# srihari-humbarwadi/retinanet-tensorflow2.x

Hardware: AMD Instinct MI355X
Metric: images/sec train, ResNet50-640 RetinaNet data-parallel step (encode + fwd + loss + bwd + clip + all-reduce + SGD/EMA); inference images/s under `infer` (higher is better)
Workload: dtype bf16; 1 GPU; ResNet50-640x640 bf16 training, 32 images/GPU (BASELINE configs[2] shard: global batch 32), resnet_initial frozen, single GPU; global_batch=32, parallelism=dp1, rccl_ranks=1, comm=torch, syncbn_messages=0

## Files before the change

retinanet-tensorflow2.x_amd/csrc/rn_conv_big.hip:

```cpp
#include "rn_conv_big_epi.h"

namespace {

constexpr int BM = 256, BN = 256, BK = 32, NW = 8, STAGES = 4;
constexpr int A_BYTES = BM * BK * 2, STAGE_BYTES = (BM + BN) * BK * 2;
constexpr int RING_BYTES = STAGES * STAGE_BYTES, PATCH_BYTES = 4096;
constexpr int LDS_BYTES = RING_BYTES + NW * PATCH_BYTES;

template <bool OUT_F32, bool HAS_RES, bool BN_BWD = false>
__global__ void __launch_bounds__(512) conv_big_kernel(const ConvArgs args) {
  extern __shared__ __attribute__((aligned(16))) char smem[];
  const int total = args.total_tiles;
  const int G = gridDim.x;
  const int tid = threadIdx.x;
  const int lane = tid & 63;
  const int wave = __builtin_amdgcn_readfirstlane(tid >> 6);
  const int wave_m = wave >> 2, wave_n = wave & 3;
  const int R = args.R, S = args.S, RS = R * S;

  int i_v = blockIdx.x;
  int i_tap = 0, i_c0 = 0;
  int i_r = 0, i_s = 0;
  int g_iss = 0;
  int i_W = 0, i_PS = 0, i_Cin = 0, i_cw = 0;
  __amdgpu_buffer_rsrc_t rs_x, rs_w;
  unsigned a_off[2], a_mask[2], b_off[2];
  const int d_row = lane >> 2, d_pos = lane & 3;

#define BIG_SETUP_ISSUE()                                                                             \
  do {                                                                                                \
    const int tile__ = (args.pad_ & 2) ? i_v : tile_of(i_v, total);      \
    int si__ = 0;                                                                                     \
    _Pragma("unroll 1") for (int i = 1; i < args.nseg; ++i)                                           \
      if (tile__ >= args.seg[i].tile_begin) si__ = i;                                                 \
    const ConvSegDev& sg__ = args.seg[si__];                                                          \
    const int lt__ = tile__ - sg__.tile_begin;                                                        \
    const int mt__ = rn_fdiv(lt__, sg__.n_tiles, rn_rcp((float)sg__.n_tiles));   \
    const int rows_t__ = sg__.rows ? sg__.rows : BM;      \
    const int m0__ = mt__ * rows_t__, n0__ = (lt__ - mt__ * sg__.n_tiles) * BN;                       \
    const int mend__ = m0__ + rows_t__ < sg__.M ? m0__ + rows_t__ : sg__.M;                           \
    i_W = sg__.W; i_PS = sg__.pix_stride; i_Cin = sg__.CinP; i_cw = sg__.cwrap;                       \
    const int H__ = sg__.H, Ktot__ = RS * i_Cin;                                                      \
    const int rows__ = sg__.Cout <= 64 ? 64 : ((sg__.Cout + 127) / 128) * 128;  \
    rs_x = __builtin_amdgcn_make_buffer_rsrc((void*)sg__.x, 0,                                        \
                                             (int)((long long)sg__.N * H__ * i_W * i_PS * 2), 0x00020000); \
    rs_w = __builtin_amdgcn_make_buffer_rsrc((void*)sg__.w, 0, (int)((long long)rows__ * Ktot__ * 2), \
                                             0x00020000);                                             \
    const float rWo__ = rn_rcp((float)sg__.Wo), rHo__ = rn_rcp((float)sg__.Ho);                 \
    _Pragma("unroll") for (int j = 0; j < 2; ++j) {                                                   \
      const int row = (j * NW + wave) * 16 + d_row;                                                   \
      const int chunk = d_pos ^ lds_swz<BK>(row);                                                     \
      const int m = m0__ + row;                                                                       \
      const int mm = m < mend__ ? m : 0;                                                              \
      int ox, oy, n;                                                                                  \
      if (args.pad_ & 1) {    \
        const int t2 = rn_fdiv(mm, sg__.Wo, rWo__);                                                   \
        ox = mm - t2 * sg__.Wo;                                                                       \
        n = rn_fdiv(t2, sg__.Ho, rHo__);                                                              \
        oy = t2 - n * sg__.Ho;                                                                        \
      } else {                                                                                        \
        ox = mm % sg__.Wo;                                                                            \
        const int t2 = mm / sg__.Wo;                                                                  \
        oy = t2 % sg__.Ho;                                                                            \
        n = t2 / sg__.Ho;                                                                             \
      }                                                                                               \
      const int iy0 = oy * args.sh - args.pt, ix0 = ox * args.sw - args.pl;                           \
      a_off[j] = (unsigned)(((((long long)n * H__ + iy0) * i_W + ix0) * i_PS + chunk * 8) * 2);       \
      unsigned mask = 0;                                                                              \
      if (m < mend__) {                                                                               \
        for (int r = 0; r < R; ++r)                                                                   \
          for (int s = 0; s < S; ++s) {                                                               \
            const bool ok = (unsigned)(iy0 + r) < (unsigned)H__ && (unsigned)(ix0 + s) < (unsigned)i_W; \
            mask |= (ok ? 1u : 0u) << (r * S + s);                                                    \
          }                                                                                           \
      }                                                                                               \
      a_mask[j] = mask;                                                                               \
      const int nrow = n0__ + row;                                                                    \
      b_off[j] = nrow < rows__ ? (unsigned)(((long long)nrow * Ktot__ + chunk * 8) * 2) : RN_OOB;     \
    }                                                                                                 \
  } while (0)

#define BIG_ISSUE_STEP()                                                                              \
  do {                                                                                                \
    const int cw__ = i_c0 < i_cw ? i_c0 : (i_c0 < 2 * i_cw ? i_c0 - i_cw : i_c0 - 2 * i_cw);          \
    const unsigned tap_off__ = (unsigned)((((long long)i_r * i_W + i_s) * i_PS + cw__) * 2);          \
    const unsigned koff__ = (unsigned)(((long long)i_tap * i_Cin + i_c0) * 2);                        \
    char* st__ = smem + (g_iss & 3) * STAGE_BYTES;                                                    \
    _Pragma("unroll") for (int j = 0; j < 2; ++j) {                                                   \
      const unsigned v__ = ((a_mask[j] >> i_tap) & 1u) ? a_off[j] + tap_off__ : RN_OOB;               \
      dma16(rs_x, st__ + (j * NW + wave) * 1024, v__);                                                \
    }                                                                                                 \
    _Pragma("unroll") for (int j = 0; j < 2; ++j)                                                     \
      dma16(rs_w, st__ + A_BYTES + (j * NW + wave) * 1024, b_off[j] == RN_OOB ? RN_OOB : b_off[j] + koff__); \
    ++g_iss;                                                                                          \
    i_c0 += BK;                                                                                       \
    if (i_c0 >= i_Cin) {                                                                              \
      i_c0 = 0;                                                                                       \
      ++i_tap;                                                                                        \
      if (++i_s == S) {                                                                               \
        i_s = 0;                                                                                      \
        ++i_r;                                                                                        \
      }                                                                                               \
      if (__builtin_expect(i_tap == RS, 0)) {                                                         \
        i_tap = i_r = i_s = 0;                                                                        \
        i_v += G;                                                                                     \
        if (i_v < total) BIG_SETUP_ISSUE();                                                           \
      }                                                                                               \
    }                                                                                                 \
  } while (0)

  int off_p0, off_w0;
  {
    const int fr = lane & 31, fh = lane >> 5;
    const int sw = (fr >> 2) & 3;
    off_p0 = (wave_m * 128 + fr) * 64 + ((0 + fh) ^ sw) * 16;
    off_w0 = A_BYTES + (wave_n * 64 + fr) * 64 + ((0 + fh) ^ sw) * 16;
  }

  f32x16_t acc[4][2];
#pragma unroll
  for (int i = 0; i < 4; ++i)
#pragma unroll
    for (int j = 0; j < 2; ++j)
#pragma unroll
      for (int r = 0; r < 16; ++r) acc[i][j][r] = 0.0f;

  bf16x8_t px0[4], wt0[2], px1[4], wt1[2];
#define BIG_READ(stage_)                                                                              \
  do {                                                                                                \
    const char* b__ = smem + (stage_) * STAGE_BYTES;                                                  \
    _Pragma("unroll") for (int j = 0; j < 2; ++j) wt0[j] = *(const bf16x8_t*)(b__ + off_w0 + j * 2048); \
    _Pragma("unroll") for (int i = 0; i < 4; ++i) px0[i] = *(const bf16x8_t*)(b__ + off_p0 + i * 2048); \
    _Pragma("unroll") for (int j = 0; j < 2; ++j) wt1[j] = *(const bf16x8_t*)(b__ + (off_w0 ^ 32) + j * 2048); \
    _Pragma("unroll") for (int i = 0; i < 4; ++i) px1[i] = *(const bf16x8_t*)(b__ + (off_p0 ^ 32) + i * 2048); \
  } while (0)
#define BIG_LOADSEG(stage_)                                                                           \
  do {                                                                                                \
    BIG_READ(stage_);                                                                                 \
    if (i_v < total) {                                                                                \
      BIG_ISSUE_STEP();                                                                               \
      asm volatile("s_waitcnt vmcnt(8)" ::: "memory");                                                \
    } else {                                                                                          \
      asm volatile("s_waitcnt vmcnt(0)" ::: "memory");                                                \
    }                                                                                                 \
    asm volatile("s_waitcnt lgkmcnt(0)" ::: "memory");                                                \
  } while (0)
#define BIG_COMPUTESEG()                                                                              \
  do {                                                                                                \
    __builtin_amdgcn_sched_barrier(0);                                                                \
    _Pragma("unroll") for (int i = 0; i < 4; ++i)                                                     \
      _Pragma("unroll") for (int j = 0; j < 2; ++j)                                                   \
        acc[i][j] = RN_MFMA_32x32x16(wt0[j], px0[i], acc[i][j], 0, 0, 0);      \
    _Pragma("unroll") for (int i = 0; i < 4; ++i)                                                     \
      _Pragma("unroll") for (int j = 0; j < 2; ++j)                                                   \
        acc[i][j] = RN_MFMA_32x32x16(wt1[j], px1[i], acc[i][j], 0, 0, 0);      \
    __builtin_amdgcn_sched_barrier(0);                                                                \
  } while (0)
#define BIG_BARRIER()                       \
  do {                                      \
    __builtin_amdgcn_s_barrier();           \
    asm volatile("" ::: "memory");          \
  } while (0)

  int c_v = blockIdx.x;
  int c_k = 0;
  int c_ksteps, c_m0, c_n0, c_si, c_mend, c_chunk0;
#define BIG_SETUP_COMPUTE()                                                                           \
  do {                                                                                                \
    const int tile__ = (args.pad_ & 2) ? c_v : tile_of(c_v, total);                                   \
    c_si = 0;                                                                                         \
    _Pragma("unroll 1") for (int i = 1; i < args.nseg; ++i)                                           \
      if (tile__ >= args.seg[i].tile_begin) c_si = i;                                                 \
    const ConvSegDev& sg__ = args.seg[c_si];                                                          \
    const int lt__ = tile__ - sg__.tile_begin;                                                        \
    const int mt__ = rn_fdiv(lt__, sg__.n_tiles, rn_rcp((float)sg__.n_tiles));   \
    const int rows_t__ = sg__.rows ? sg__.rows : BM;                                                  \
    c_m0 = mt__ * rows_t__;                                                                           \
    c_mend = c_m0 + rows_t__ < sg__.M ? c_m0 + rows_t__ : sg__.M;                                     \
    c_chunk0 = mt__ * 2;                                                                              \
    c_n0 = (lt__ - mt__ * sg__.n_tiles) * BN;                                                         \
    c_ksteps = RS * (sg__.CinP / BK);                                                                 \
    c_k = 0;                                                                                          \
  } while (0)

  auto epilogue = [&]() __attribute__((always_inline)) {
    big_epilogue<OUT_F32, HAS_RES, BN_BWD>(acc, args, c_si, c_m0, c_n0, wave, smem + RING_BYTES + wave * PATCH_BYTES,
                                           BigEpiSrc(), c_mend, c_chunk0);
  };

  BIG_SETUP_ISSUE();
  BIG_SETUP_COMPUTE();
  big_acc_init<OUT_F32, HAS_RES>(acc, args, c_si, c_n0, wave);
#pragma unroll 1
  for (int t = 0; t < 3 && i_v < total; ++t) BIG_ISSUE_STEP();
  if (g_iss >= 3) asm volatile("s_waitcnt vmcnt(4)" ::: "memory");
  else asm volatile("s_waitcnt vmcnt(0)" ::: "memory");
  BIG_BARRIER();
  BIG_LOADSEG(0);
  if (wave_m == 1) BIG_BARRIER();

#define BIG_TILE_END()                                       \
  if (__builtin_expect(c_k == c_ksteps, 0)) {               \
    epilogue();                                             \
    if (c_v + G >= total) break;                            \
    c_v += G;                                               \
    BIG_SETUP_COMPUTE();                                    \
    big_acc_init<OUT_F32, HAS_RES>(acc, args, c_si, c_n0, wave); \
  }
  int g = 0;
#pragma unroll 1
  while (true) {
    BIG_COMPUTESEG();
    ++c_k;
    if (wave_m == 0) BIG_BARRIER();
    BIG_TILE_END();
    if (wave_m == 1) BIG_BARRIER();
    ++g;
    BIG_LOADSEG(g & 3);
    BIG_BARRIER();
  }
#undef BIG_TILE_END
#undef BIG_SETUP_COMPUTE
#undef BIG_BARRIER
#undef BIG_COMPUTESEG
#undef BIG_LOADSEG
#undef BIG_READ
#undef BIG_ISSUE_STEP
#undef BIG_SETUP_ISSUE
}

}

int rn_launch_conv_big(const ConvArgs& a, bool out_f32, const rn_launch_opts& opts, hipStream_t st) {
  static unsigned long long attr_set = 0;
  if (RN_ATTRS_NEEDED(attr_set)) {
    RN_CHECK_HIP(hipFuncSetAttribute((const void*)conv_big_kernel<false, false>,
                                     hipFuncAttributeMaxDynamicSharedMemorySize, LDS_BYTES));
    RN_CHECK_HIP(hipFuncSetAttribute((const void*)conv_big_kernel<false, true>,
                                     hipFuncAttributeMaxDynamicSharedMemorySize, LDS_BYTES));
    RN_CHECK_HIP(hipFuncSetAttribute((const void*)conv_big_kernel<true, false>,
                                     hipFuncAttributeMaxDynamicSharedMemorySize, LDS_BYTES));
    RN_CHECK_HIP(hipFuncSetAttribute((const void*)conv_big_kernel<true, true>,
                                     hipFuncAttributeMaxDynamicSharedMemorySize, LDS_BYTES));
    RN_CHECK_HIP(hipFuncSetAttribute((const void*)conv_big_kernel<false, false, true>,
                                     hipFuncAttributeMaxDynamicSharedMemorySize, LDS_BYTES));
    RN_ATTRS_DONE(attr_set);
  }
  const int grid = rn_persistent_grid(a.total_tiles, rn_num_cus(), opts);
  bool has_res = false;
  for (int i = 0; i < a.nseg; ++i) has_res = has_res || a.seg[i].residual != nullptr;
  const dim3 g3(grid), b3(512);
  if (a.seg[0].bn_y) {
    hipLaunchKernelGGL((conv_big_kernel<false, false, true>), g3, b3, LDS_BYTES, st, a);
  } else if (out_f32) {
    if (has_res) hipLaunchKernelGGL((conv_big_kernel<true, true>), g3, b3, LDS_BYTES, st, a);
    else hipLaunchKernelGGL((conv_big_kernel<true, false>), g3, b3, LDS_BYTES, st, a);
  } else {
    if (has_res) hipLaunchKernelGGL((conv_big_kernel<false, true>), g3, b3, LDS_BYTES, st, a);
    else hipLaunchKernelGGL((conv_big_kernel<false, false>), g3, b3, LDS_BYTES, st, a);
  }
  RN_CHECK_LAUNCH();
  return RN_OK;
}
```

retinanet-tensorflow2.x_amd/csrc/rn_conv_dispatch.hip:

```cpp
#include <algorithm>
#include <map>
#include <mutex>
#include <tuple>

#include "rn_conv_dev.h"

extern "C" int rn_conv_cout_pad(int Cout) { return Cout <= 64 ? 64 : (int)rn_align_up((size_t)Cout, 128); }
extern "C" int rn_conv_cin_pad(int Cin) { return Cin <= 32 ? 32 : (int)rn_align_up((size_t)Cin, 64); }
extern "C" int rn_conv_pair_rows(int Cout) { return Cout > 0 ? 128 * ((Cout + 63) / 64) : 0; }

struct ConvPlanSeg {
  int cols, cols_pad;
  int terms, cin_pad;
  long long M;
  int n_tiles, tile_begin;
  int bn_row_blocks;
};

struct ConvPlan {
  int kid;
  int BM, BN;
  int BK;
  int bal_rows;
  bool deal;
  bool fast_div;
  int order[RN_CONV_MAX_SEGMENTS];
  long long total_tiles;
  int min_depth;
  int split_parts;
  long long ws_bytes;
  ConvPlanSeg seg[RN_CONV_MAX_SEGMENTS];
};

static long long seg_tiles(const ConvPlanSeg& s, int rows, int width) { return rn_cdiv(s.M, rows) * rn_cdiv(s.cols_pad, width); }
static long long conv_tiles(const ConvPlan& pl, int nseg, int rows, int width) {
  long long t = 0;
  for (int i = 0; i < nseg; ++i) t += seg_tiles(pl.seg[i], rows, width);
  return t;
}

static bool conv_halo_fits(const rn_conv_problem* p, int BM) {
  if (p->opts.conv_no_halo) return false;
  if (p->R != 3 || p->S != 3 || p->stride_h != 1 || p->stride_w != 1 || p->pad_top != 1 || p->pad_left != 1)
    return false;
  static std::mutex mu;
  static std::map<std::tuple<int, int, int, int>, int> patch_px;
  for (int i = 0; i < p->num_segments; ++i) {
    const rn_conv_segment& s = p->seg[i];
    if (s.Ho != s.H || s.Wo != s.W || s.Cin % 32 != 0) return false;
    if ((long long)s.N * s.H * s.W >= (1ll << 22)) return false;
    std::lock_guard<std::mutex> lock(mu);
    const auto key = std::make_tuple(s.N, s.H, s.W, BM);
    auto it = patch_px.find(key);
    if (it == patch_px.end()) it = patch_px.emplace(key, rn_conv_halo_patch_pixels(s.N, s.H, s.W, rn_conv_halo_pitch(s.W), BM)).first;
    if (it->second > rn_conv_halo_capacity(BM)) return false;
  }
  return true;
}

static int splitk_parts(int total, int min_chunks, int G0, long long* bytes) {
  const int L = total % G0;
  if (bytes) *bytes = 0;
  if (L == 0 || L > 511 || min_chunks < 8) return 1;
  int S = G0 / L;
  if (S > min_chunks / 4) S = min_chunks / 4;
  if (S > 4) S = 4;
  if (S < 2) return 1;
  if (bytes) *bytes = RN_SPLITK_HEADER_BYTES + (long long)L * S * RN_SPLITK_SLOT_BYTES;
  return S;
}

static void rn_splitk_plan(ConvArgs& a, int min_chunks, void* ws, long long ws_bytes, const rn_launch_opts& opts) {
  const int total = a.total_tiles;
  a.split_f = total; a.split_s = 1; a.vtotal = total; a.pad2_ = 0; a.ws = nullptr;
  const int G0 = rn_persistent_grid(0x7fffffff, rn_num_cus(), opts);
  const int L = total % G0;
  int S = ws ? splitk_parts(total, min_chunks, G0, nullptr) : 1;
  while (S >= 2 && RN_SPLITK_HEADER_BYTES + (long long)L * S * RN_SPLITK_SLOT_BYTES > ws_bytes) --S;
  if (S < 2) return;
  a.split_f = total - L; a.split_s = S; a.vtotal = L * S; a.ws = (float*)ws;
}

extern "C" size_t rn_conv_splitk_workspace_max_bytes(void) { return RN_SPLITK_HEADER_BYTES + 256ull * RN_SPLITK_SLOT_BYTES; }

static int conv_big_balanced_rows(const rn_conv_problem* p, const ConvPlanSeg& s) {
  if (p->num_segments != 1 || p->R != 1 || p->S != 1 || p->stride_h != 1 || p->stride_w != 1) return 0;
  if (p->opts.conv_tile || p->opts.conv_big_min_tiles || p->opts.max_workgroups || p->splitk_ws) return 0;
  if (s.terms * s.cin_pad > 512) return 0;
  const int n_tiles = (int)rn_cdiv(s.cols_pad, 256);
  const int G = rn_persistent_grid(0x7fffffff, rn_num_cus(), p->opts);
  const long long T = seg_tiles(s, 256, 256);
  if (T <= 0 || G <= 0) return 0;
  const long long rounds = rn_cdiv(T, G);
  const long long m_tiles = rounds * G / n_tiles;
  if (m_tiles < 1) return 0;
  long long rows = rn_cdiv(s.M, m_tiles);
  rows = (rows + 3) / 4 * 4;
  if (rows < 64 || rows > 236) return 0;
  return (int)rows;
}

#define RN_SPLIT128_MIN_STEPS 4
static int conv128_split_parts(const rn_launch_opts& opts, long long tiles, int ksteps, int BN, long long ws_bytes) {
  if (opts.conv_tile == 1 || tiles < 1 || tiles > 4096) return 1;
  const int target = opts.splitk_target_blocks > 0 ? opts.splitk_target_blocks : rn_num_cus() * 3 / 4;
  int S = target / (int)tiles;
  if (S > ksteps / RN_SPLIT128_MIN_STEPS) S = ksteps / RN_SPLIT128_MIN_STEPS;
  if (S > 8) S = 8;
  const long long slot = 128ll * BN * 4;
  while (S >= 2 && RN_SPLITK_HEADER_BYTES + tiles * S * slot > ws_bytes) --S;
  return S >= 2 ? S : 1;
}

static bool conv_plan(const rn_conv_problem* p, bool assume_ws, ConvPlan& pl) {
  if (!p || p->num_segments < 1 || p->num_segments > RN_CONV_MAX_SEGMENTS) return false;
  const int nseg = p->num_segments;
  const rn_launch_opts& o = p->opts;

  bool all_wide = true, all_128 = true, all_128s_or_64 = true, one_col = true;
  bool epi_ok = true;
  long long dmin = 1ll << 60, dmax = 0;
  pl.min_depth = 0x7fffffff;
  pl.fast_div = true;
  for (int i = 0; i < nseg; ++i) {
    const rn_conv_segment& s = p->seg[i];
    ConvPlanSeg& d = pl.seg[i];
    d.cols = s.w_pair ? rn_conv_pair_rows(s.Cout) : s.Cout;
    d.cols_pad = rn_conv_cout_pad(d.cols);
    d.terms = s.w_terms > 1 ? s.w_terms : 1;
    d.cin_pad = rn_conv_cin_pad(s.Cin);
    d.M = (long long)s.N * s.Ho * s.Wo;
    all_wide = all_wide && d.cols_pad >= 256;
    all_128 = all_128 && d.cols_pad == 128;
    all_128s_or_64 = all_128s_or_64 && (d.cols_pad % 128 == 0 || d.cols_pad == 64);
    one_col = one_col && d.cols_pad <= 256;
    epi_ok = epi_ok && s.Cout % (p->out_dtype == RN_DT_F32 && s.w_pair ? 4 : 8) == 0 && !(s.bias && s.residual);
    const int depth = d.terms * d.cin_pad;
    pl.min_depth = depth < pl.min_depth ? depth : pl.min_depth;
    const long long depth_all = (long long)p->R * p->S * d.cin_pad * d.terms;
    dmin = depth_all < dmin ? depth_all : dmin;
    dmax = depth_all > dmax ? depth_all : dmax;
    pl.fast_div = pl.fast_div && d.M < (1 << 22);
  }
  const int cin0 = pl.seg[0].cin_pad;
  pl.BK = (cin0 % 64 != 0 || (long long)p->R * p->S * cin0 <= 256) ? 32 : 64;

  const bool use_big = o.conv_tile != 1 && o.conv_tile != 3 && all_wide && epi_ok &&
                       (o.conv_tile == 2 || conv_tiles(pl, nseg, 256, 256) >= (o.conv_big_min_tiles > 0 ? o.conv_big_min_tiles : 192));
  if (use_big) {
    if (!conv_halo_fits(p, 256)) pl.kid = 1;
    else pl.kid = (o.conv_tile == 0 && o.conv_big_min_tiles == 0 && conv_halo_fits(p, 512)) ? 3 : 2;
  } else {
    const bool halo512 = o.conv_tile != 1 && !o.conv_no_halo && (o.conv_tile == 3 ? all_128s_or_64 : all_128) && epi_ok &&
                         (o.conv_tile >= 2 || conv_tiles(pl, nseg, 512, 128) >= (o.conv_big_min_tiles > 0 ? o.conv_big_min_tiles : 128)) &&
                         conv_halo_fits(p, 512);
    pl.kid = halo512 ? 3 : 0;
  }

  pl.bal_rows = 0;
  if (pl.kid == 0) {
    pl.BM = 128;
    pl.BN = pl.seg[0].cols_pad <= 64 ? 64 : 128;
    if (pl.BN == 128 && o.conv_tile != 1 && 2 * conv_tiles(pl, nseg, 128, 128) <= rn_num_cus()) pl.BN = 64;
  } else if (pl.kid == 3) {
    pl.BM = 512; pl.BN = 128;
  } else {
    pl.BM = 256; pl.BN = 256;
    if (pl.kid == 1) pl.bal_rows = conv_big_balanced_rows(p, pl.seg[0]);
  }

  for (int i = 0; i < nseg; ++i) pl.order[i] = i;
  pl.deal = pl.kid == 1 && nseg > 1 && one_col && dmax >= 2 * dmin;
  if (pl.deal)
    std::stable_sort(pl.order, pl.order + nseg, [&](int x, int y) {
      return pl.seg[x].cin_pad * pl.seg[x].terms > pl.seg[y].cin_pad * pl.seg[y].terms;
    });
  const int rows = pl.bal_rows ? pl.bal_rows : pl.BM;
  pl.total_tiles = 0;
  for (int ii = 0; ii < nseg; ++ii) {
    ConvPlanSeg& d = pl.seg[pl.order[ii]];
    d.n_tiles = (int)rn_cdiv(d.cols_pad, pl.BN);
    d.tile_begin = (int)pl.total_tiles;
    d.bn_row_blocks = (int)(pl.bal_rows ? 2 * rn_cdiv(d.M, rows) : (rows / 128) * rn_cdiv(d.M, rows));
    pl.total_tiles += seg_tiles(d, rows, pl.BN);
  }

  pl.split_parts = 1;
  pl.ws_bytes = 0;
  if (pl.kid == 0) {
    if (p->splitk_ws || assume_ws) {
      const long long avail = p->splitk_ws ? p->splitk_ws_bytes : (long long)rn_conv_splitk_workspace_max_bytes();
      pl.split_parts = conv128_split_parts(o, pl.total_tiles, p->R * p->S * (pl.min_depth / pl.BK), pl.BN, avail);
    }
    if (pl.split_parts >= 2) pl.ws_bytes = RN_SPLITK_HEADER_BYTES + pl.total_tiles * pl.split_parts * 128 * pl.BN * 4;
  } else if (pl.kid == 2) {
    splitk_parts((int)pl.total_tiles, pl.min_depth / 32, rn_persistent_grid(0x7fffffff, rn_num_cus(), o), &pl.ws_bytes);
  }
  return true;
}

extern "C" size_t rn_conv_splitk_workspace_bytes(const rn_conv_problem* p) {
  ConvPlan pl;
  return conv_plan(p, true, pl) ? (size_t)pl.ws_bytes : 0;
}

extern "C" int rn_conv_kernel_id(const rn_conv_problem* p) {
  ConvPlan pl;
  return conv_plan(p, false, pl) ? pl.kid : -1;
}

extern "C" int rn_conv_bn_row_blocks(const rn_conv_problem* p, int segment) {
  ConvPlan pl;
  if (!conv_plan(p, false, pl) || segment < 0 || segment >= p->num_segments) return 0;
  return pl.seg[segment].bn_row_blocks;
}

extern "C" int rn_conv_tile_rows(const rn_conv_problem* p) {
  ConvPlan pl;
  return conv_plan(p, false, pl) ? pl.BM : 0;
}

static int conv_validate(const rn_conv_problem* p, const ConvPlan& pl) {
  RN_CHECK_ARG(p->R >= 1 && p->S >= 1 && p->R * p->S <= 32, "rn_conv2d_nhwc_fwd: R*S=%d > 32", p->R * p->S);
  RN_CHECK_ARG(p->stride_h >= 1 && p->stride_w >= 1, "rn_conv2d_nhwc_fwd: bad stride");
  RN_CHECK_ARG(p->out_dtype == RN_DT_BF16 || p->out_dtype == RN_DT_F32, "rn_conv2d_nhwc_fwd: bad out_dtype");
  if (const int orc = rn_validate_launch_opts(p->opts, "rn_conv2d_nhwc_fwd")) return orc;
  for (int ii = 0; ii < p->num_segments; ++ii) {
    const int i = pl.order[ii];
    const rn_conv_segment& s = p->seg[i];
    RN_CHECK_ARG(s.x && s.w && s.y, "rn_conv2d_nhwc_fwd: segment %d has a null tensor", i);
    RN_CHECK_ARG(s.N > 0 && s.H > 0 && s.W > 0 && s.Ho > 0 && s.Wo > 0 && s.Cout > 0 && s.Cin > 0,
                 "rn_conv2d_nhwc_fwd: segment %d bad shape", i);
    RN_CHECK_ARG(s.Cin % 8 == 0 && pl.seg[i].cin_pad % pl.BK == 0,
                 "rn_conv2d_nhwc_fwd: segment %d Cin=%d must be a multiple of 8 (K step %d)", i, s.Cin, pl.BK);
    RN_CHECK_ARG(s.pix_stride % 4 == 0 && s.pix_stride > 0,
                 "rn_conv2d_nhwc_fwd: segment %d pix_stride=%d must be a positive multiple of 4", i, s.pix_stride);
    RN_CHECK_ARG(s.Cout % 4 == 0, "rn_conv2d_nhwc_fwd: segment %d Cout=%d not a multiple of 4", i, s.Cout);
    RN_CHECK_ARG((pl.seg[i].cols_pad <= 64) == (pl.seg[0].cols_pad <= 64), "rn_conv2d_nhwc_fwd: segments mix Cout tile widths");
    RN_CHECK_ARG(!s.w_pair || (pl.kid != 0 && p->out_dtype == RN_DT_F32 && s.w_terms <= 1 && !s.scale && !s.shift &&
                               !s.residual && !s.bn_partial),
                 "rn_conv2d_nhwc_fwd: segment %d: w_pair needs an f32 launch without scale / shift / residual that the 256- / "
                 "512-row kernels take (rn_conv_kernel_id() != 0)", i);
    RN_CHECK_ARG(((uintptr_t)s.x | (uintptr_t)s.w | (uintptr_t)s.y | (uintptr_t)s.residual) % 16 == 0,
                 "rn_conv2d_nhwc_fwd: segment %d tensors must be 16-byte aligned", i);
    RN_CHECK_ARG(pl.seg[i].M < (1ll << 31) && (long long)s.N * s.H * s.W * s.pix_stride * 2 < (1ll << 31),
                 "rn_conv2d_nhwc_fwd: segment %d input exceeds the 2 GiB buffer-addressing limit", i);
    if (s.bn_bwd_y) {
      RN_CHECK_ARG(s.bn_partial && s.bn_bwd_fwd && p->out_dtype == RN_DT_BF16 && !s.scale && !s.shift && !s.bias &&
                       !s.residual && p->act == RN_ACT_NONE && s.Cout % 8 == 0 && (uintptr_t)s.bn_bwd_y % 16 == 0,
                   "rn_conv2d_nhwc_fwd: segment %d: bn_bwd_y needs bn_partial + bn_bwd_fwd on a plain bf16 launch", i);
    }
    RN_CHECK_ARG((s.bn_bwd_y != nullptr) == (p->seg[0].bn_bwd_y != nullptr),
                 "rn_conv2d_nhwc_fwd: bn_bwd_y must be set on all segments or none");
    RN_CHECK_ARG(pl.seg[i].terms <= 3, "rn_conv2d_nhwc_fwd: segment %d w_terms=%d (1..3)", i, s.w_terms);
  }
  RN_CHECK_ARG(p->splitk_ws == nullptr || ((uintptr_t)p->splitk_ws % 16 == 0 && p->splitk_ws_bytes >= 0),
               "rn_conv2d_nhwc_fwd: splitk_ws must be 16-byte aligned");
  return RN_OK;
}

extern "C" int rn_conv2d_nhwc_fwd(const rn_conv_problem* p, void* stream) {
  RN_CHECK_ARG(p != nullptr, "rn_conv2d_nhwc_fwd: null problem");
  RN_CHECK_ARG(p->num_segments >= 1 && p->num_segments <= RN_CONV_MAX_SEGMENTS,
               "rn_conv2d_nhwc_fwd: num_segments=%d", p->num_segments);
  ConvPlan pl;
  conv_plan(p, false, pl);
  if (const int rc = conv_validate(p, pl)) return rc;

  ConvArgs a;
  a.R = p->R; a.S = p->S; a.sh = p->stride_h; a.sw = p->stride_w; a.pt = p->pad_top; a.pl = p->pad_left;
  a.act = p->act; a.nseg = p->num_segments;
  a.total_tiles = (int)pl.total_tiles;
  a.pad_ = pl.kid <= 1 ? (pl.fast_div ? 1 : 0) | (pl.deal ? 2 : 0) : 0;
  a.split_f = a.vtotal = a.total_tiles; a.split_s = 1; a.pad2_ = 0; a.ws = nullptr;
  for (int ii = 0; ii < p->num_segments; ++ii) {
    const rn_conv_segment& s = p->seg[pl.order[ii]];
    const ConvPlanSeg& ps = pl.seg[pl.order[ii]];
    ConvSegDev& d = a.seg[ii];
    d.x = (const uint16_t*)s.x; d.w = (const uint16_t*)s.w; d.y = s.y;
    d.scale = s.scale; d.shift = s.shift; d.residual = (const uint16_t*)s.residual;
    d.bn_partial = s.bn_partial;
    d.bn_y = (const uint16_t*)s.bn_bwd_y;
    d.bn_fwd = s.bn_bwd_fwd;
    d.bias = s.bias;
    d.N = s.N; d.H = s.H; d.W = s.W; d.Cin = s.Cin; d.pix_stride = s.pix_stride;
    d.Ho = s.Ho; d.Wo = s.Wo; d.Cout = ps.cols;
    d.pair_cout = s.w_pair ? s.Cout : 0;
    d.rows = pl.bal_rows;
    d.M = (int)ps.M;
    d.tile_begin = ps.tile_begin;
    d.n_tiles = ps.n_tiles;
    d.cwrap = ps.cin_pad;
    d.CinP = ps.terms * ps.cin_pad;
    d.halo_pitch = s.W + 1;
  }

  hipStream_t st = (hipStream_t)stream;
  const bool f32 = p->out_dtype == RN_DT_F32;
  switch (pl.kid) {
    case 3: return rn_launch_conv_halo(a, f32, p->opts, st, 4);
    case 2:
      rn_splitk_plan(a, pl.min_depth / 32, p->splitk_ws, p->splitk_ws_bytes, p->opts);
      return rn_launch_conv_halo(a, f32, p->opts, st);
    case 1: return rn_launch_conv_big(a, f32, p->opts, st);
  }
  if (pl.split_parts >= 2) {
    a.split_s = pl.split_parts; a.vtotal = a.total_tiles * pl.split_parts; a.ws = (float*)p->splitk_ws;
  }
  return rn_launch_conv128(a, pl.BN, pl.BK, f32, pl.split_parts >= 2, st);
}
```

retinanet-tensorflow2.x_amd/csrc/rn_core.hip:

```cpp
#include "rn_common.h"
#include <string.h>
#include <new>

static thread_local char g_rn_err[512] = "";

void rn_set_error(const char* fmt, ...) {
  va_list ap;
  va_start(ap, fmt);
  vsnprintf(g_rn_err, sizeof(g_rn_err), fmt, ap);
  va_end(ap);
}

extern "C" const char* rn_last_error(void) { return g_rn_err; }

extern "C" int rn_abi_version(void) { return 15; }

extern "C" int rn_storage_dtype(void) {
#ifdef RN_F16
  return 1;
#else
  return 0;
#endif
}

extern "C" int rn_device_ok(void) {
  int n = 0;
  if (hipGetDeviceCount(&n) != hipSuccess || n <= 0) {
    (void)hipGetLastError();
    return 0;
  }
  hipDeviceProp_t p;
  if (hipGetDeviceProperties(&p, 0) != hipSuccess) return 0;
  return strncmp(p.gcnArchName, "gfx950", 6) == 0 ? 1 : 0;
}

struct rn_handle {
  int device;
  int num_cus;
  rn_launch_opts opts;
  void* comm[4];
};

static int rn_check_opts(const rn_launch_opts& o, const char* who) {
  RN_CHECK_ARG(o.conv_tile >= 0 && o.conv_tile <= 3, "%s: conv_tile=%d (0..3)", who, o.conv_tile);
  RN_CHECK_ARG(o.wgrad_kernel >= 0 && o.wgrad_kernel <= 3, "%s: wgrad_kernel=%d (0..3)", who, o.wgrad_kernel);
  RN_CHECK_ARG(o.reserved_cus >= 0 && o.reserved_cus <= 128, "%s: reserved_cus=%d out of range (0..128)", who,
               o.reserved_cus);
  RN_CHECK_ARG(o.max_workgroups >= 0 && o.conv_big_min_tiles >= 0 && o.wgrad_target_blocks >= 0 && o.splitk_target_blocks >= 0,
               "%s: negative max_workgroups / conv_big_min_tiles / wgrad_target_blocks / splitk_target_blocks", who);
#ifndef RN_PROBES
  RN_CHECK_ARG(o.ablate == 0, "%s: ablate=%d: the timing variants exist in the probe build (-DRN_PROBES) only", who, o.ablate);
#endif
  return RN_OK;
}
int rn_validate_launch_opts(const rn_launch_opts& o, const char* who) { return rn_check_opts(o, who); }

extern "C" int rn_create(int device_id, rn_handle** out) {
  RN_CHECK_ARG(out != nullptr, "rn_create: null out");
  *out = nullptr;
  int n = 0;
  RN_CHECK_HIP(hipGetDeviceCount(&n));
  RN_CHECK_ARG(device_id >= 0 && device_id < n, "rn_create: device %d of %d", device_id, n);
  hipDeviceProp_t p;
  RN_CHECK_HIP(hipGetDeviceProperties(&p, device_id));
  RN_CHECK_ARG(strncmp(p.gcnArchName, "gfx950", 6) == 0, "rn_create: device %d is %s, this library is gfx950 only",
               device_id, p.gcnArchName);
  rn_handle* h = new (std::nothrow) rn_handle();
  if (!h) {
    rn_set_error("rn_create: out of host memory");
    return RN_ENOMEM;
  }
  h->device = device_id;
  h->num_cus = p.multiProcessorCount;
  memset(&h->opts, 0, sizeof(h->opts));
  for (auto& c : h->comm) c = nullptr;
  *out = h;
  return RN_OK;
}

extern "C" int rn_destroy(rn_handle* h) {
  if (!h) return RN_OK;
  int rc = RN_OK;
  for (auto& c : h->comm)
    if (c) {
      const int r = rn_comm_destroy(c);
      if (r != RN_OK) rc = r;
      c = nullptr;
    }
  delete h;
  return rc;
}

extern "C" int rn_handle_device(const rn_handle* h) { return h ? h->device : RN_EINVAL; }
extern "C" int rn_handle_num_cus(const rn_handle* h) { return h ? h->num_cus : RN_EINVAL; }

extern "C" int rn_handle_set_launch_opts(rn_handle* h, const rn_launch_opts* opts) {
  RN_CHECK_ARG(h && opts, "rn_handle_set_launch_opts: null argument");
  const int rc = rn_check_opts(*opts, "rn_handle_set_launch_opts");
  if (rc != RN_OK) return rc;
  h->opts = *opts;
  return RN_OK;
}

extern "C" int rn_handle_get_launch_opts(const rn_handle* h, rn_launch_opts* opts) {
  RN_CHECK_ARG(h && opts, "rn_handle_get_launch_opts: null argument");
  *opts = h->opts;
  return RN_OK;
}

extern "C" int rn_handle_comm_init(rn_handle* h, int slot, const void* unique_id, int rank, int world) {
  RN_CHECK_ARG(h && slot >= 0 && slot < 4, "rn_handle_comm_init: bad handle / slot %d (0..3)", slot);
  RN_CHECK_ARG(h->comm[slot] == nullptr, "rn_handle_comm_init: slot %d already holds a communicator", slot);
  return rn_comm_init(unique_id, rank, world, &h->comm[slot]);
}

extern "C" int rn_handle_comm_destroy(rn_handle* h, int slot) {
  RN_CHECK_ARG(h && slot >= 0 && slot < 4, "rn_handle_comm_destroy: bad handle / slot %d (0..3)", slot);
  if (!h->comm[slot]) return RN_OK;
  void* c = h->comm[slot];
  h->comm[slot] = nullptr;
  return rn_comm_destroy(c);
}

extern "C" void* rn_handle_comm(const rn_handle* h, int slot) {
  return (h && slot >= 0 && slot < 4) ? h->comm[slot] : nullptr;
}

int rn_persistent_grid(int work_items, int num_cu, const rn_launch_opts& o) {
  int g = num_cu - o.reserved_cus;
  if (o.max_workgroups > 0 && o.max_workgroups < g) g = o.max_workgroups;
  if (g < 1) g = 1;
  return work_items < g ? work_items : g;
}

int rn_device_slot() {
  int dev = 0;
  if (hipGetDevice(&dev) != hipSuccess || dev < 0) return 0;
  return dev & 63;
}

int rn_num_cus() {
  static int cus[64] = {0};
  int dev = 0;
  if (hipGetDevice(&dev) != hipSuccess || dev < 0 || dev >= 64) return 256;
  if (!cus[dev]) {
    hipDeviceProp_t prop;
    cus[dev] = (hipGetDeviceProperties(&prop, dev) == hipSuccess && prop.multiProcessorCount > 0)
                   ? prop.multiProcessorCount : 256;
  }
  return cus[dev];
}
```

Baseline: 1132 images/s.

## Add panel-walk 1x1 conv kernel that keeps activation panel resident and streams weights

Adds a new persistent kernel for 1x1 stride-1 convolutions with residual, wide output (>=512 channels) and shallow input (<=256). Each workgroup loads a 128-row activation panel into LDS once and streams weight tiles per wave through a double-buffered ring across all output-column passes. This replaces the 256x256 tile scheme, which reloads the activations for every column tile. The dispatcher picks it by default for residual-carrying 1x1 expand convs and balances the panel rows across CUs. Each wave gets a smaller MFMA tile and weights are re-read per panel, and the kernel relies on the custom wait-count choreography being correct.

```diff
diff --git a/retinanet-tensorflow2.x_amd/csrc/rn_conv_big.hip b/retinanet-tensorflow2.x_amd/csrc/rn_conv_big.hip
--- a/retinanet-tensorflow2.x_amd/csrc/rn_conv_big.hip
+++ b/retinanet-tensorflow2.x_amd/csrc/rn_conv_big.hip
@@ -229,6 +229,125 @@
 #undef BIG_SETUP_ISSUE
 }
 
+constexpr int PANEL_BYTES = 128 * 256 * 2, WSTAGE_BYTES = 64 * BK * 2, WRING_BYTES = NW * 2 * WSTAGE_BYTES;
+static_assert(PANEL_BYTES + WRING_BYTES + NW * PATCH_BYTES <= LDS_BYTES, "panel walk: LDS budget");
+
+template <bool HAS_RES, bool BN_BWD = false>
+__global__ void __launch_bounds__(512) conv_big_panel_kernel(const ConvArgs args) {
+  extern __shared__ __attribute__((aligned(16))) char smem[];
+  const int n_panels = args.total_tiles;
+  const int G = gridDim.x;
+  const int tid = threadIdx.x;
+  const int lane = tid & 63;
+  const int wave = __builtin_amdgcn_readfirstlane(tid >> 6);
+  const ConvSegDev& sg = args.seg[0];
+  const int M = sg.M, K = sg.CinP, KS = K / BK;
+  const int prow = sg.rows ? sg.rows : 128;
+  const int wrows = sg.Cout <= 64 ? 64 : ((sg.Cout + 127) / 128) * 128;
+  const int NP = (wrows + 511) / 512;
+  const __amdgpu_buffer_rsrc_t rs_x = __builtin_amdgcn_make_buffer_rsrc(
+      (void*)sg.x, 0, (int)((long long)M * sg.pix_stride * 2), 0x00020000);
+  const __amdgpu_buffer_rsrc_t rs_w = __builtin_amdgcn_make_buffer_rsrc((void*)sg.w, 0, (int)((long long)wrows * K * 2), 0x00020000);
+  const int d_row = lane >> 2, d_pos = lane & 3;
+  const int d_chunk = d_pos ^ lds_swz<BK>(d_row);
+  char* const panel = smem;
+  char* const ring = smem + PANEL_BYTES + wave * 2 * WSTAGE_BYTES;
+  char* const patch = smem + PANEL_BYTES + WRING_BYTES + wave * PATCH_BYTES;
+
+  const int my_panels = (n_panels - (int)blockIdx.x + G - 1) / G;
+  const int T = my_panels * NP * KS;
+
+  auto issue_panel = [&](int v) __attribute__((always_inline)) {
+    const int m0 = tile_of(v, n_panels) * prow;
+    const int mend = m0 + prow < M ? m0 + prow : M;
+    const int m = m0 + wave * 16 + d_row;
+    const unsigned base = (unsigned)(((long long)m * sg.pix_stride + d_chunk * 8) * 2);
+#pragma unroll 1
+    for (int s = 0; s < KS; ++s) {
+      const int c0 = s * BK;
+      const int cw = c0 < sg.cwrap ? c0 : (c0 < 2 * sg.cwrap ? c0 - sg.cwrap : c0 - 2 * sg.cwrap);
+      dma16(rs_x, panel + s * (128 * BK * 2) + wave * 1024, m < mend ? base + (unsigned)(cw * 2) : RN_OOB);
+    }
+  };
+  int w_pass = 0, w_s = 0, w_iss = 0;
+  auto issue_weights = [&]() __attribute__((always_inline)) {
+    char* st = ring + (w_iss & 1) * WSTAGE_BYTES;
+#pragma unroll
+    for (int j = 0; j < 4; ++j) {
+      const int n = w_pass * 512 + wave * 64 + j * 16 + d_row;
+      const unsigned off = (unsigned)(((long long)n * K + w_s * BK + d_chunk * 8) * 2);
+      dma16(rs_w, st + j * 1024, n < wrows ? off : RN_OOB);
+    }
+    ++w_iss;
+    if (++w_s == KS) {
+      w_s = 0;
+      if (++w_pass == NP) w_pass = 0;
+    }
+  };
+
+  int off_p0, off_w0;
+  {
+    const int fr = lane & 31, fh = lane >> 5;
+    const int sw = (fr >> 2) & 3;
+    off_p0 = fr * 64 + ((0 + fh) ^ sw) * 16;
+    off_w0 = fr * 64 + ((0 + fh) ^ sw) * 16;
+  }
+  f32x16_t acc[4][2];
+  bf16x8_t px0[4], wt0[2], px1[4], wt1[2];
+
+  issue_panel(blockIdx.x);
+  issue_weights();
+  if (T > 1) issue_weights();
+  int t = 0;
+#pragma unroll 1
+  for (int v = blockIdx.x; v < n_panels; v += G) {
+    const int pidx = tile_of(v, n_panels);
+    const int m0 = pidx * prow;
+    const int mend = m0 + prow < M ? m0 + prow : M;
+    asm volatile("s_waitcnt vmcnt(0)" ::: "memory");
+    __builtin_amdgcn_s_barrier();
+    asm volatile("" ::: "memory");
+#pragma unroll 1
+    for (int p = 0; p < NP; ++p) {
+      big_acc_init<false, HAS_RES, 1>(acc, args, 0, p * 512, wave);
+#pragma unroll 1
+      for (int s = 0; s < KS; ++s) {
+        if (t + 1 < T) asm volatile("s_waitcnt vmcnt(4)" ::: "memory");
+        else asm volatile("s_waitcnt vmcnt(0)" ::: "memory");
+        const char* wb = ring + (t & 1) * WSTAGE_BYTES;
+        const char* pb = panel + s * (128 * BK * 2);
+#pragma unroll
+        for (int j = 0; j < 2; ++j) wt0[j] = *(const bf16x8_t*)(wb + off_w0 + j * 2048);
+#pragma unroll
+        for (int i = 0; i < 4; ++i) px0[i] = *(const bf16x8_t*)(pb + off_p0 + i * 2048);
+#pragma unroll
+        for (int j = 0; j < 2; ++j) wt1[j] = *(const bf16x8_t*)(wb + (off_w0 ^ 32) + j * 2048);
+#pragma unroll
+        for (int i = 0; i < 4; ++i) px1[i] = *(const bf16x8_t*)(pb + (off_p0 ^ 32) + i * 2048);
+        asm volatile("s_waitcnt lgkmcnt(0)" ::: "memory");
+        if (t + 2 < T) issue_weights();
+        __builtin_amdgcn_sched_barrier(0);
+#pragma unroll
+        for (int i = 0; i < 4; ++i)
+#pragma unroll
+          for (int j = 0; j < 2; ++j) acc[i][j] = RN_MFMA_32x32x16(wt0[j], px0[i], acc[i][j], 0, 0, 0);
+#pragma unroll
+        for (int i = 0; i < 4; ++i)
+#pragma unroll
+          for (int j = 0; j < 2; ++j) acc[i][j] = RN_MFMA_32x32x16(wt1[j], px1[i], acc[i][j], 0, 0, 0);
+        __builtin_amdgcn_sched_barrier(0);
+        ++t;
+      }
+      if (p == NP - 1) {
+        __builtin_amdgcn_s_barrier();
+        asm volatile("" ::: "memory");
+        if (v + G < n_panels) issue_panel(v + G);
+      }
+      big_epilogue<false, HAS_RES, BN_BWD, false, 1>(acc, args, 0, m0, p * 512, wave, patch, BigEpiSrc(), mend, pidx);
+    }
+  }
+}
+
 }
 
 int rn_launch_conv_big(const ConvArgs& a, bool out_f32, const rn_launch_opts& opts, hipStream_t st) {
@@ -244,7 +363,21 @@
                                      hipFuncAttributeMaxDynamicSharedMemorySize, LDS_BYTES));
     RN_CHECK_HIP(hipFuncSetAttribute((const void*)conv_big_kernel<false, false, true>,
                                      hipFuncAttributeMaxDynamicSharedMemorySize, LDS_BYTES));
+    RN_CHECK_HIP(hipFuncSetAttribute((const void*)conv_big_panel_kernel<false>,
+                                     hipFuncAttributeMaxDynamicSharedMemorySize, LDS_BYTES));
+    RN_CHECK_HIP(hipFuncSetAttribute((const void*)conv_big_panel_kernel<true>,
+                                     hipFuncAttributeMaxDynamicSharedMemorySize, LDS_BYTES));
+    RN_CHECK_HIP(hipFuncSetAttribute((const void*)conv_big_panel_kernel<false, true>,
+                                     hipFuncAttributeMaxDynamicSharedMemorySize, LDS_BYTES));
     RN_ATTRS_DONE(attr_set);
+  }
+  if (a.pad_ & 4) {
+    const dim3 gp(rn_persistent_grid(a.total_tiles, rn_num_cus(), opts)), bp(512);
+    if (a.seg[0].bn_y) hipLaunchKernelGGL((conv_big_panel_kernel<false, true>), gp, bp, LDS_BYTES, st, a);
+    else if (a.seg[0].residual) hipLaunchKernelGGL((conv_big_panel_kernel<true>), gp, bp, LDS_BYTES, st, a);
+    else hipLaunchKernelGGL((conv_big_panel_kernel<false>), gp, bp, LDS_BYTES, st, a);
+    RN_CHECK_LAUNCH();
+    return RN_OK;
   }
   const int grid = rn_persistent_grid(a.total_tiles, rn_num_cus(), opts);
   bool has_res = false;
diff --git a/retinanet-tensorflow2.x_amd/csrc/rn_conv_dispatch.hip b/retinanet-tensorflow2.x_amd/csrc/rn_conv_dispatch.hip
--- a/retinanet-tensorflow2.x_amd/csrc/rn_conv_dispatch.hip
+++ b/retinanet-tensorflow2.x_amd/csrc/rn_conv_dispatch.hip
@@ -22,6 +22,7 @@
   int BM, BN;
   int BK;
   int bal_rows;
+  bool panel;
   bool deal;
   bool fast_div;
   int order[RN_CONV_MAX_SEGMENTS];
@@ -97,6 +98,30 @@
   long long rows = rn_cdiv(s.M, m_tiles);
   rows = (rows + 3) / 4 * 4;
   if (rows < 64 || rows > 236) return 0;
+  return (int)rows;
+}
+
+static bool conv_big_panel_fits(const rn_conv_problem* p, const ConvPlanSeg& s) {
+  if (p->num_segments != 1 || p->R != 1 || p->S != 1 || p->stride_h != 1 || p->stride_w != 1) return false;
+  if (p->pad_top != 0 || p->pad_left != 0 || p->out_dtype != RN_DT_BF16 || p->seg[0].w_pair) return false;
+  if (p->seg[0].Ho != p->seg[0].H || p->seg[0].Wo != p->seg[0].W) return false;
+  return s.terms * s.cin_pad <= 256 && s.cols_pad >= 512;
+}
+static bool conv_big_panel_wanted(const rn_conv_problem* p, const ConvPlanSeg& s) {
+  if (!conv_big_panel_fits(p, s)) return false;
+  if (p->opts.conv_tile == 4) return true;
+  if (p->opts.conv_tile || p->opts.conv_big_min_tiles || p->opts.max_workgroups || p->splitk_ws) return false;
+  return p->seg[0].residual != nullptr;
+}
+static int conv_big_panel_rows(const rn_conv_problem* p, const ConvPlanSeg& s) {
+  if (p->opts.conv_big_min_tiles || p->opts.max_workgroups) return 0;
+  const int G = rn_persistent_grid(0x7fffffff, rn_num_cus(), p->opts);
+  const long long P = rn_cdiv(s.M, 128);
+  if (P <= 0 || G <= 0) return 0;
+  const long long panels = rn_cdiv(P, G) * G;
+  long long rows = rn_cdiv(s.M, panels);
+  rows = (rows + 3) / 4 * 4;
+  if (rows < 64 || rows > 118) return 0;
   return (int)rows;
 }
 
@@ -145,28 +170,36 @@
   const int cin0 = pl.seg[0].cin_pad;
   pl.BK = (cin0 % 64 != 0 || (long long)p->R * p->S * cin0 <= 256) ? 32 : 64;
 
-  const bool use_big = o.conv_tile != 1 && o.conv_tile != 3 && all_wide && epi_ok &&
-                       (o.conv_tile == 2 || conv_tiles(pl, nseg, 256, 256) >= (o.conv_big_min_tiles > 0 ? o.conv_big_min_tiles : 192));
+  const int conv_tile = o.conv_tile == 4 ? 2 : o.conv_tile;
+  const bool use_big = conv_tile != 1 && conv_tile != 3 && all_wide && epi_ok &&
+                       (conv_tile == 2 || conv_tiles(pl, nseg, 256, 256) >= (o.conv_big_min_tiles > 0 ? o.conv_big_min_tiles : 192));
   if (use_big) {
     if (!conv_halo_fits(p, 256)) pl.kid = 1;
-    else pl.kid = (o.conv_tile == 0 && o.conv_big_min_tiles == 0 && conv_halo_fits(p, 512)) ? 3 : 2;
+    else pl.kid = (conv_tile == 0 && o.conv_big_min_tiles == 0 && conv_halo_fits(p, 512)) ? 3 : 2;
   } else {
-    const bool halo512 = o.conv_tile != 1 && !o.conv_no_halo && (o.conv_tile == 3 ? all_128s_or_64 : all_128) && epi_ok &&
-                         (o.conv_tile >= 2 || conv_tiles(pl, nseg, 512, 128) >= (o.conv_big_min_tiles > 0 ? o.conv_big_min_tiles : 128)) &&
+    const bool halo512 = conv_tile != 1 && !o.conv_no_halo && (conv_tile == 3 ? all_128s_or_64 : all_128) && epi_ok &&
+                         (conv_tile >= 2 || conv_tiles(pl, nseg, 512, 128) >= (o.conv_big_min_tiles > 0 ? o.conv_big_min_tiles : 128)) &&
                          conv_halo_fits(p, 512);
     pl.kid = halo512 ? 3 : 0;
   }
 
   pl.bal_rows = 0;
+  pl.panel = false;
   if (pl.kid == 0) {
     pl.BM = 128;
     pl.BN = pl.seg[0].cols_pad <= 64 ? 64 : 128;
-    if (pl.BN == 128 && o.conv_tile != 1 && 2 * conv_tiles(pl, nseg, 128, 128) <= rn_num_cus()) pl.BN = 64;
+    if (pl.BN == 128 && conv_tile != 1 && 2 * conv_tiles(pl, nseg, 128, 128) <= rn_num_cus()) pl.BN = 64;
   } else if (pl.kid == 3) {
     pl.BM = 512; pl.BN = 128;
   } else {
     pl.BM = 256; pl.BN = 256;
-    if (pl.kid == 1) pl.bal_rows = conv_big_balanced_rows(p, pl.seg[0]);
+    pl.panel = pl.kid == 1 && conv_big_panel_wanted(p, pl.seg[0]);
+    if (pl.panel) {
+      pl.BM = 128;
+      pl.bal_rows = conv_big_panel_rows(p, pl.seg[0]);
+    } else if (pl.kid == 1) {
+      pl.bal_rows = conv_big_balanced_rows(p, pl.seg[0]);
+    }
   }
 
   for (int i = 0; i < nseg; ++i) pl.order[i] = i;
@@ -181,8 +214,8 @@
     ConvPlanSeg& d = pl.seg[pl.order[ii]];
     d.n_tiles = (int)rn_cdiv(d.cols_pad, pl.BN);
     d.tile_begin = (int)pl.total_tiles;
-    d.bn_row_blocks = (int)(pl.bal_rows ? 2 * rn_cdiv(d.M, rows) : (rows / 128) * rn_cdiv(d.M, rows));
-    pl.total_tiles += seg_tiles(d, rows, pl.BN);
+    d.bn_row_blocks = (int)(pl.panel ? rn_cdiv(d.M, rows) : pl.bal_rows ? 2 * rn_cdiv(d.M, rows) : (rows / 128) * rn_cdiv(d.M, rows));
+    pl.total_tiles += pl.panel ? rn_cdiv(d.M, rows) : seg_tiles(d, rows, pl.BN);
   }
 
   pl.split_parts = 1;
@@ -271,7 +304,7 @@
   a.R = p->R; a.S = p->S; a.sh = p->stride_h; a.sw = p->stride_w; a.pt = p->pad_top; a.pl = p->pad_left;
   a.act = p->act; a.nseg = p->num_segments;
   a.total_tiles = (int)pl.total_tiles;
-  a.pad_ = pl.kid <= 1 ? (pl.fast_div ? 1 : 0) | (pl.deal ? 2 : 0) : 0;
+  a.pad_ = pl.kid <= 1 ? (pl.fast_div ? 1 : 0) | (pl.deal ? 2 : 0) | (pl.panel ? 4 : 0) : 0;
   a.split_f = a.vtotal = a.total_tiles; a.split_s = 1; a.pad2_ = 0; a.ws = nullptr;
   for (int ii = 0; ii < p->num_segments; ++ii) {
     const rn_conv_segment& s = p->seg[pl.order[ii]];
diff --git a/retinanet-tensorflow2.x_amd/csrc/rn_core.hip b/retinanet-tensorflow2.x_amd/csrc/rn_core.hip
--- a/retinanet-tensorflow2.x_amd/csrc/rn_core.hip
+++ b/retinanet-tensorflow2.x_amd/csrc/rn_core.hip
@@ -41,8 +41,8 @@
   void* comm[4];
 };
 
-static int rn_check_opts(const rn_launch_opts& o, const char* who) {
-  RN_CHECK_ARG(o.conv_tile >= 0 && o.conv_tile <= 3, "%s: conv_tile=%d (0..3)", who, o.conv_tile);
+static int rn_check_opts(const rn_launch_opts& o, const char* who, int per_launch = 0) {
+  RN_CHECK_ARG(o.conv_tile >= 0 && o.conv_tile <= 3 + per_launch, "%s: conv_tile=%d (0..%d)", who, o.conv_tile, 3 + per_launch);
   RN_CHECK_ARG(o.wgrad_kernel >= 0 && o.wgrad_kernel <= 3, "%s: wgrad_kernel=%d (0..3)", who, o.wgrad_kernel);
   RN_CHECK_ARG(o.reserved_cus >= 0 && o.reserved_cus <= 128, "%s: reserved_cus=%d out of range (0..128)", who,
                o.reserved_cus);
@@ -53,7 +53,7 @@
 #endif
   return RN_OK;
 }
-int rn_validate_launch_opts(const rn_launch_opts& o, const char* who) { return rn_check_opts(o, who); }
+int rn_validate_launch_opts(const rn_launch_opts& o, const char* who) { return rn_check_opts(o, who, 1); }
 
 extern "C" int rn_create(int device_id, rn_handle** out) {
   RN_CHECK_ARG(out != nullptr, "rn_create: null out");
```

After: 1132 images/s, median of 2. About the same (-0.0%).
